# yisol/IDM-VTON

Hardware: AMD Instinct MI355X
Metric: try-on images/sec at 768x1024, 30 DDIM steps, guidance 2.0 (higher is better)
Workload: dtype bf16; 1 GPU; BASELINE.json configs[1]: 768x1024, 30 steps, batch 2/GPU, guidance 2.0, bf16 storage / fp32 accumulate, scheduler ddim, hipGraph on, GarmentNet batched over 6 timesteps, GarmentNet(block b+1)||TryonNet(block b) two-stream overlap on; images_per_call=2, parallelism=dp1 (image shards, one start-up RCCL weight broadcast), rccl_ranks=1

## Files before the change

idm-vton_amd/csrc/gemm_body.cuh:

```cuda
#pragma once
#include <type_traits>
#if !defined(__gfx950__) && !defined(__gfx942__) && defined(__HIP_DEVICE_COMPILE__)
#error "gemm_body.cuh: the counted vmcnt pipeline is written for gfx94x/gfx950 (stores counted in vmcnt)"
#endif
#include "common.cuh"
#include "gemm_common.cuh"

template <typename T, int BN, int BM, int WN, int WM, int ST, bool V1, bool LIN, bool PF, bool TR, bool XA = false>
__device__ __forceinline__ void gemm_body(const GemmParams& p, char* smem, const int m0, const int n0) {
    typedef typename VT<T>::v8 v8;
    typedef typename VT<T>::v4 v4;
    constexpr int NW = WN * WM;
    constexpr int SN = BN / WN, SM = BM / WM;
    constexpr int NI = SN / 32, MI = SM / 32;
    constexpr int WBYTES = BN * 128, XBYTES = BM * 128;
    constexpr int PW_ = BN / 8, PX_ = BM / 8;
    constexpr bool UNEVEN = (PW_ % NW != 0) || (PX_ % NW != 0);
    constexpr int WI = (PW_ + NW - 1) / NW, XI = (PX_ + NW - 1) / NW;
    static_assert(BN % 8 == 0 && BM % 8 == 0 && WN * SN == BN && WM * SM == BM && NI * 32 == SN && MI * 32 == SM, "tile / wave-count mismatch");
    static_assert(!UNEVEN || (V1 && ST == 2), "round-robin piece assignment needs the two-stage ring");
    char* sW = smem;
    char* sX = smem + ST * WBYTES;

    const int lane = threadIdx.x & 63;
    const int wave = uniform(threadIdx.x >> 6);
    const int wn = wave / WM, wm = wave % WM;
    const int u = lane >> 5, l31 = lane & 31;

    const int lrow = lane >> 3, lslot = lane & 7;
    auto wj = [&](int i) { return UNEVEN ? wave + i * NW : wave * WI + i; };
    auto xj = [&](int i) { return UNEVEN ? wave + i * NW : wave * XI + i; };
    uint32_t w_off[WI];
#pragma unroll
    for (int i = 0; i < WI; ++i) {
        const int R = wj(i) * 8 + lrow;
        const int c = lslot ^ ((R >> 1) & 7);
        w_off[i] = ((uint32_t)(n0 + R) * (uint32_t)p.Ktot + c * 8) * 2u;
    }
    int x_pix[XI], x_oy[XI], x_ox[XI], x_c8[XI];
    uint32_t x_off[XI];
    const int HoWo = p.Ho * p.Wo;
    auto kbyte = [&](int t) -> uint32_t { return (uint32_t)t * 128u; };
#pragma unroll
    for (int i = 0; i < XI; ++i) {
        const int R = xj(i) * 8 + lrow;
        const int m = m0 + R;
        x_c8[i] = (lslot ^ ((R >> 1) & 7)) * 8;
        if constexpr (LIN) {
            x_off[i] = m < p.M ? ((uint32_t)m * (uint32_t)p.seg[0].pitch + p.seg[0].coff + x_c8[i]) * 2u : OOB_SENTINEL;
        } else if (m < p.M) {
            const int b = m / HoWo, rem = m - b * HoWo;
            const int oy = rem / p.Wo, ox = rem - oy * p.Wo;
            x_pix[i] = b * p.Hi * p.Wi; x_oy[i] = oy * p.stride; x_ox[i] = ox * p.stride;
        } else {
            x_pix[i] = 0; x_oy[i] = -(1 << 28); x_ox[i] = 0;
        }
    }
    const __amdgpu_buffer_rsrc_t rs_w = make_rsrc(p.w, p.w_bytes);
    const __amdgpu_buffer_rsrc_t rs_x0 = make_rsrc(p.seg[0].ptr, p.seg[0].bytes);
    const int hin = p.ups ? p.Ho : p.Hi, win = p.ups ? p.Wo : p.Wi;

    int si = 0, kseg = 0;
    auto issue = [&](int t, int buf) {
        char* dW = sW + buf * WBYTES;
        char* dX = sX + buf * XBYTES;
#pragma unroll
        for (int i = 0; i < WI; ++i) {
            if (UNEVEN && wj(i) >= PW_) continue;
            dma16(rs_w, dW + wj(i) * 1024, w_off[i] + kbyte(t));
        }
        if constexpr (LIN) {
#pragma unroll
            for (int i = 0; i < XI; ++i) {
                if (UNEVEN && xj(i) >= PX_) continue;
                dma16(rs_x0, dX + xj(i) * 1024, x_off[i] + kbyte(t));
            }
        } else {
            const idmvton_seg sg = p.seg[si];
            const __amdgpu_buffer_rsrc_t rs_x = make_rsrc(sg.ptr, sg.bytes);
#pragma unroll
            for (int i = 0; i < XI; ++i) {
                if (UNEVEN && xj(i) >= PX_) continue;
                int iy = x_oy[i] + sg.dy, ix = x_ox[i] + sg.dx;
                const bool ok = (unsigned)iy < (unsigned)hin && (unsigned)ix < (unsigned)win;
                if (p.ups) { iy >>= 1; ix >>= 1; }
                const uint32_t off = ((uint32_t)(x_pix[i] + iy * p.Wi + ix) * (uint32_t)sg.pitch + sg.coff + kseg + x_c8[i]) * 2u;
                dma16(rs_x, dX + xj(i) * 1024, ok ? off : OOB_SENTINEL);
            }
            kseg += 64;
            if (kseg >= sg.len) { kseg = 0; ++si; }
        }
    };

    idmvton_seg sgc = p.seg[0];
    __amdgpu_buffer_rsrc_t rs_xc = rs_x0;
    auto issue_part = [&](int t, int buf, int s) {
        constexpr int LPT_ = WI + XI;
        char* dW = sW + buf * WBYTES;
        char* dX = sX + buf * XBYTES;
        if constexpr (!LIN) {
            if (s == 0) { sgc = p.seg[si]; rs_xc = make_rsrc(sgc.ptr, sgc.bytes); }
        }
#pragma unroll
        for (int j = 0; j < LPT_; ++j) {
            if ((j & 3) != s) continue;
            if (j < WI) {
                if (UNEVEN && wj(j) >= PW_) continue;
                dma16(rs_w, dW + wj(j) * 1024, w_off[j] + kbyte(t));
            } else {
                const int i = j - WI;
                if (UNEVEN && xj(i) >= PX_) continue;
                if constexpr (LIN) dma16(rs_x0, dX + xj(i) * 1024, x_off[i] + kbyte(t));
                else {
                    int iy = x_oy[i] + sgc.dy, ix = x_ox[i] + sgc.dx;
                    const bool ok = (unsigned)iy < (unsigned)hin && (unsigned)ix < (unsigned)win;
                    if (p.ups) { iy >>= 1; ix >>= 1; }
                    const uint32_t off = ((uint32_t)(x_pix[i] + iy * p.Wi + ix) * (uint32_t)sgc.pitch + sgc.coff + kseg + x_c8[i]) * 2u;
                    dma16(rs_xc, dX + xj(i) * 1024, ok ? off : OOB_SENTINEL);
                }
            }
        }
        if constexpr (!LIN) {
            if (s == 3) { kseg += 64; if (kseg >= sgc.len) { kseg = 0; ++si; } }
        }
    };

    int a_row[NI], a_swz[NI], b_row[MI], b_swz[MI];
#pragma unroll
    for (int ni = 0; ni < NI; ++ni) { const int r = wn * SN + ni * 32 + l31; a_row[ni] = r * 128; a_swz[ni] = (r >> 1) & 7; }
#pragma unroll
    for (int mi = 0; mi < MI; ++mi) { const int r = wm * SM + mi * 32 + l31; b_row[mi] = r * 128; b_swz[mi] = (r >> 1) & 7; }

    f32x16 acc[NI][MI];
#pragma unroll
    for (int ni = 0; ni < NI; ++ni)
#pragma unroll
        for (int mi = 0; mi < MI; ++mi)
#pragma unroll
            for (int r = 0; r < 16; ++r) acc[ni][mi][r] = 0.f;

    auto frag_a = [&](const char* bW, int s, int ni) { return *(const v8*)(bW + a_row[ni] + (((2 * s + u) ^ a_swz[ni]) << 4)); };
    auto frag_b = [&](const char* bX, int s, int mi) { return *(const v8*)(bX + b_row[mi] + (((2 * s + u) ^ b_swz[mi]) << 4)); };
    auto compute = [&](int buf, bool spread = false, int t_next = 0, int buf_next = 0) {
        const char* bW = sW + buf * WBYTES;
        const char* bX = sX + buf * XBYTES;
        if constexpr (!PF) {
#pragma unroll
            for (int s = 0; s < 4; ++s) {
                v8 a[NI], b[MI];
#pragma unroll
                for (int ni = 0; ni < NI; ++ni) a[ni] = frag_a(bW, s, ni);
#pragma unroll
                for (int mi = 0; mi < MI; ++mi) b[mi] = frag_b(bX, s, mi);
                if constexpr (V1) {
                    if (spread) issue_part(t_next, buf_next, s);
                    __builtin_amdgcn_sched_barrier(0);
                }
#pragma unroll
                for (int ni = 0; ni < NI; ++ni)
#pragma unroll
                    for (int mi = 0; mi < MI; ++mi)
                        acc[ni][mi] = TR ? VT<T>::mfma(b[mi], a[ni], acc[ni][mi]) : VT<T>::mfma(a[ni], b[mi], acc[ni][mi]);
            }
        } else {
            v8 a[2][NI], b[2][MI];
#pragma unroll
            for (int ni = 0; ni < NI; ++ni) a[0][ni] = frag_a(bW, 0, ni);
#pragma unroll
            for (int mi = 0; mi < MI; ++mi) b[0][mi] = frag_b(bX, 0, mi);
#pragma unroll
            for (int s = 0; s < 4; ++s) {
                if (s < 3) {
#pragma unroll
                    for (int ni = 0; ni < NI; ++ni) a[(s + 1) & 1][ni] = frag_a(bW, s + 1, ni);
#pragma unroll
                    for (int mi = 0; mi < MI; ++mi) b[(s + 1) & 1][mi] = frag_b(bX, s + 1, mi);
                }
                if (spread) issue_part(t_next, buf_next, s);
                __builtin_amdgcn_sched_barrier(0);
#pragma unroll
                for (int ni = 0; ni < NI; ++ni)
#pragma unroll
                    for (int mi = 0; mi < MI; ++mi)
                        acc[ni][mi] = TR ? VT<T>::mfma(b[s & 1][mi], a[s & 1][ni], acc[ni][mi])
                                         : VT<T>::mfma(a[s & 1][ni], b[s & 1][mi], acc[ni][mi]);
                __builtin_amdgcn_sched_barrier(0);
            }
        }
    };

    v8 xkf[XA ? XA_NK : 1];
    int xa_b = 0, xa_h = 0;
    if constexpr (XA) {
        static_assert(NI == 2 && !TR, "fused cross-attention: one 64-channel head per wave");
        const int mw = m0 + wm * SM;
        xa_b = (mw < p.M ? mw : p.M - 1) / p.xa.tokens;
        xa_h = (n0 + wn * SN) >> 6;
        xattn_load_k<T>(p.xa, xa_b, xa_h, lane, xkf);
    }
    const int nt = p.Ktot >> 6;
    if constexpr (!V1) {
        issue(0, 0);
        for (int t = 0; t < nt; ++t) {
            asm volatile("s_waitcnt vmcnt(0)" ::: "memory");
            __syncthreads();
            if (t + 1 < nt) issue(t + 1, (t + 1) & 1);
            compute(t & 1);
        }
    } else {
        constexpr int LPT = WI + XI;
        static_assert((ST - 2) * LPT < 64, "vmcnt immediate is 6 bits");
#pragma unroll
        for (int s = 0; s < ST - 1; ++s)
            if (s < nt) issue(s, s);
        int cbuf = 0, ibuf = ST - 1;
        for (int t = 0; t < nt; ++t) {
            if (t + ST - 2 < nt) wait_vmcnt<(ST - 2) * LPT>(); else wait_vmcnt<0>();
            __builtin_amdgcn_s_barrier();
            asm volatile("" ::: "memory");
            compute(cbuf, t + ST - 1 < nt, t + ST - 1, ibuf);
            cbuf = cbuf + 1 == ST ? 0 : cbuf + 1;
            ibuf = ibuf + 1 == ST ? 0 : ibuf + 1;
        }
    }

    if constexpr (XA) {
        v8 xvf[XA_NV];
        xattn_load_v<T>(p.xa, xa_b, xa_h, lane, xvf);
        xattn_compute<T, MI>(p.xa, p.M, acc, m0 + wm * SM, lane, xkf, xvf);
    }
    gemm_epilogue<T, NI, MI, SN, SM, TR>(p, acc, m0, n0, wn, wm, lane);
}

template <typename T, int BN, int BM, int WN, int WM, int ST, bool V1, bool LIN, int OCC, bool PFX = false>
__global__ __launch_bounds__(WN * WM * 64, OCC) void gemm_conv_kernel(const GemmParams p) {
    __shared__ __attribute__((aligned(1024))) char smem[ST * (BN + BM) * 128];
    const int wg = xcd_remap(blockIdx.x, p.tiles_m * p.tiles_n);
    int tm, tn;
    if constexpr (!V1) { tm = wg / p.tiles_n; tn = wg - tm * p.tiles_n; }
    else {
        const int GM = p.gm > 0 ? p.gm : 1024 / BM;
        const int width = GM * p.tiles_n;
        const int grp = wg / width, rem = wg - grp * width;
        const int first = grp * GM;
        const int gsz = p.tiles_m - first < GM ? p.tiles_m - first : GM;
        tn = rem / gsz; tm = first + (rem - tn * gsz);
    }
    const int m0 = tm * BM, n0 = tn * BN;
    if constexpr (BN == 320) {
        gemm_body<T, BN, BM, WN, WM, ST, V1, LIN, OCC == 1 || PFX, false>(p, smem, m0, n0);
    } else {
        if (p.vt != nullptr && n0 >= p.vt_n0) gemm_body<T, BN, BM, WN, WM, ST, V1, LIN, OCC == 1 || PFX, true>(p, smem, m0, n0);
        else gemm_body<T, BN, BM, WN, WM, ST, V1, LIN, OCC == 1 || PFX, false>(p, smem, m0, n0);
    }
}

template <typename T, int BN, int BM, int WN, int WM, int ST, int OCC>
__global__ __launch_bounds__(WN * WM * 64, OCC) void gemm_xattn_kernel(const GemmParams p) {
    __shared__ __attribute__((aligned(1024))) char smem[ST * (BN + BM) * 128];
    const int wg = xcd_remap(blockIdx.x, p.tiles_m * p.tiles_n);
    const int GM = p.gm > 0 ? p.gm : 1024 / BM;
    const int width = GM * p.tiles_n;
    const int grp = wg / width, rem = wg - grp * width;
    const int first = grp * GM;
    const int gsz = p.tiles_m - first < GM ? p.tiles_m - first : GM;
    const int tn = rem / gsz, tm = first + (rem - tn * gsz);
    gemm_body<T, BN, BM, WN, WM, ST, true, true, OCC == 1, false, true>(p, smem, tm * BM, tn * BN);
}

template <typename T, int BN, int BM, int WN, int WM, int ST, bool V1, int OCC, bool PFX = false>
static void launch_cfg(const GemmParams& p0, bool lin, hipStream_t st) {
    GemmParams p = p0;
    p.gm = V1 ? idmvton_choose_gm(p.tiles_m, p.tiles_n, BM, BN, p.Ktot) : 0;
    const dim3 grid(p.tiles_n * p.tiles_m), block(WN * WM * 64);
    if constexpr (V1) {
        if (lin) { hipLaunchKernelGGL((gemm_conv_kernel<T, BN, BM, WN, WM, ST, true, true, OCC, PFX>), grid, block, 0, st, p); return; }
    }
    hipLaunchKernelGGL((gemm_conv_kernel<T, BN, BM, WN, WM, ST, V1, false, OCC, PFX>), grid, block, 0, st, p);
}


int gemm_tiles_v0(const GemmParams& p, bool bf16, int bn, int bm, bool lin, hipStream_t st);
int gemm_tiles_v1(const GemmParams& p, bool bf16, int bn, int bm, bool lin, hipStream_t st);
int gemm_tiles_v2(const GemmParams& p, bool bf16, int bn, int bm, bool lin, hipStream_t st);
int gemm_tiles_w8(const GemmParams& p, bool bf16, int bn, int bm, int form, bool lin, hipStream_t st);
int gemm_tiles_xattn(const GemmParams& p, bool bf16, int bn, int bm, int w8, hipStream_t st);
int launch_gemm_lin(const GemmParams& p, bool bf16, int bm, int form, int grid_cap, hipStream_t st);
```

idm-vton_amd/csrc/gemm_common.cuh:

```cuda
#pragma once
#include "common.cuh"
#include "xattn.cuh"

struct GemmParams {
    const void* w; uint32_t w_bytes; int N; int Ktot;
    int nseg; idmvton_seg seg[IDMVTON_MAX_SEG];
    int M, Ho, Wo, Hi, Wi, stride, ups;
    void* out; int ldo;
    const void* bias; const void* rowbias; int rowbias_ld; int rows_per_group;
    const void* res; int ldr;
    int mode;
    void* vt; int vt_n0; int vt_tokens; int vt_perm;
    int colscale_n; float colscale;
    int tiles_m, tiles_n;
    int gm;
    int wide;
    int res32, out32;
    int bias32;
    int out8; float o8_scale, vt8_scale;
    XAttnParams xa;
};

int idmvton_choose_gm(int tiles_m, int tiles_n, int bm, int bn, int K);

template <int N> __device__ __forceinline__ void wait_vmcnt() { asm volatile("s_waitcnt vmcnt(%0)" ::"n"(N) : "memory"); }

__device__ __forceinline__ void swap_cols8(const f32x16& c, const int gp, float (&v)[8]) {
#pragma unroll
    for (int j = 0; j < 4; ++j) {
        const auto r = __builtin_amdgcn_permlane32_swap(__float_as_uint(c[8 * gp + j]), __float_as_uint(c[8 * gp + 4 + j]), false, false);
        v[j] = __uint_as_float(r[0]);
        v[4 + j] = __uint_as_float(r[1]);
    }
}

template <typename T, int NI, int MI, int SN, int SM, bool TR>
__device__ __forceinline__ void gemm_epilogue(const GemmParams& p, f32x16 (&acc)[NI][MI], const int m0, const int n0, const int wn, const int wm,
                                              const int lane) {
    typedef typename VT<T>::v4 v4;
    typedef typename VT<T>::v8 v8;
    const int u = lane >> 5, l31 = lane & 31;
    const T* bias = (const T*)p.bias;
    if constexpr (TR) {
        if (p.out8) {
            uint8_t* vt = (uint8_t*)p.vt;
            const int Cv = p.N - p.vt_n0;
#pragma unroll
            for (int ni = 0; ni < NI; ++ni) {
                const int n = n0 + wn * SN + ni * 32 + l31;
                if (n >= p.N) continue;
                const float bv = bias ? (float)bias[n] : 0.f;
#pragma unroll
                for (int mi = 0; mi < MI; ++mi) {
                    const int m = m0 + wm * SM + mi * 32;
                    if (m >= p.M) continue;
                    const int b = m / p.vt_tokens;
                    const int tok = m - b * p.vt_tokens;
                    int4 o;
                    int w[4];
#pragma unroll
                    for (int g = 0; g < 4; ++g)
                        w[g] = pack4_fp8(clamp448((acc[ni][mi][4 * g] + bv) * p.vt8_scale), clamp448((acc[ni][mi][4 * g + 1] + bv) * p.vt8_scale),
                                         clamp448((acc[ni][mi][4 * g + 2] + bv) * p.vt8_scale), clamp448((acc[ni][mi][4 * g + 3] + bv) * p.vt8_scale));
                    o.x = w[0]; o.y = w[1]; o.z = w[2]; o.w = w[3];
                    *(int4*)(vt + ((size_t)(b * Cv + n - p.vt_n0) * p.vt_tokens + (tok & ~63) + 32 * u + ((tok >> 1) & 16))) = o;
                }
            }
            return;
        }
        if (p.vt_perm) {
            T* vt = (T*)p.vt;
            const int Cv = p.N - p.vt_n0;
#pragma unroll
            for (int ni = 0; ni < NI; ++ni) {
                const int n = n0 + wn * SN + ni * 32 + l31;
                if (n >= p.N) continue;
                const float bv = bias ? (float)bias[n] : 0.f;
#pragma unroll
                for (int mi = 0; mi < MI; ++mi)
#pragma unroll
                    for (int gp = 0; gp < 2; ++gp) {
                        const int m = m0 + wm * SM + mi * 32 + 16 * gp;
                        if (m >= p.M) continue;
                        const int b = m / p.vt_tokens;
                        const int tok = m - b * p.vt_tokens + 8 * u;
                        v8 o;
#pragma unroll
                        for (int j = 0; j < 8; ++j) o[j] = (T)(acc[ni][mi][8 * gp + j] + bv);
                        *(v8*)(vt + ((size_t)(b * Cv + n - p.vt_n0) * p.vt_tokens + tok)) = o;
                    }
            }
            return;
        }
        T* vt = (T*)p.vt;
        const int Cv = p.N - p.vt_n0;
#pragma unroll
        for (int ni = 0; ni < NI; ++ni) {
            const int n = n0 + wn * SN + ni * 32 + l31;
            if (n >= p.N) continue;
            const float bv = bias ? (float)bias[n] : 0.f;
#pragma unroll
            for (int mi = 0; mi < MI; ++mi)
#pragma unroll
                for (int g = 0; g < 4; ++g) {
                    const int m = m0 + wm * SM + mi * 32 + 8 * g + 4 * u;
                    if (m >= p.M) continue;
                    const int b = m / p.vt_tokens;
                    int tok = m - b * p.vt_tokens;
                    if (p.vt_perm) tok = (tok & ~12) | ((tok & 4) << 1) | ((tok & 8) >> 1);
                    v4 o;
#pragma unroll
                    for (int j = 0; j < 4; ++j) o[j] = (T)(acc[ni][mi][4 * g + j] + bv);
                    *(v4*)(vt + ((size_t)(b * Cv + n - p.vt_n0) * p.vt_tokens + tok)) = o;
                }
        }
        return;
    }
    T* out = (T*)p.out;
    const T* res = (const T*)p.res;
    const T* rowbias = (const T*)p.rowbias;
    if (p.wide) {
#pragma unroll
        for (int mi = 0; mi < MI; ++mi) {
            const int m = m0 + wm * SM + mi * 32 + l31;
            if (m >= p.M) continue;
            const T* rb = rowbias ? rowbias + (size_t)(m / p.rows_per_group) * p.rowbias_ld : nullptr;
            if (p.mode == IDMVTON_EPI_GEGLU) {
                if constexpr (NI % 2 == 0) {
#pragma unroll
                    for (int pr = 0; pr < NI / 2; ++pr)
#pragma unroll
                        for (int gp = 0; gp < 2; ++gp) {
                            float h[8], gt[8];
                            swap_cols8(acc[2 * pr][mi], gp, h);
                            swap_cols8(acc[2 * pr + 1][mi], gp, gt);
                            const int nh = n0 + wn * SN + pr * 64 + 16 * gp + 8 * u;
                            if (nh + 32 >= p.N) continue;
                            const int jo = ((n0 + wn * SN + pr * 64) >> 1) + 16 * gp + 8 * u;
                            if (bias) {
                                const v8 bh = *(const v8*)(bias + nh), bg = *(const v8*)(bias + nh + 32);
#pragma unroll
                                for (int j = 0; j < 8; ++j) { h[j] += (float)bh[j]; gt[j] += (float)bg[j]; }
                            }
                            v8 o;
#pragma unroll
                            for (int j = 0; j < 8; ++j) o[j] = (T)(h[j] * gelu_erf(gt[j]));
                            *(v8*)(out + (size_t)m * p.ldo + jo) = o;
                        }
                }
                continue;
            }
#pragma unroll
            for (int ni = 0; ni < NI; ++ni) {
#pragma unroll
                for (int gp = 0; gp < 2; ++gp) {
                    float v[8];
                    swap_cols8(acc[ni][mi], gp, v);
                    const int n = n0 + wn * SN + ni * 32 + 16 * gp + 8 * u;
                    if (n >= p.N) continue;
                    if (bias) {
                        if (p.bias32) {
                            const float4* bp = (const float4*)((const float*)p.bias + n);
                            const float4 b0 = bp[0], b1 = bp[1];
                            v[0] += b0.x; v[1] += b0.y; v[2] += b0.z; v[3] += b0.w;
                            v[4] += b1.x; v[5] += b1.y; v[6] += b1.z; v[7] += b1.w;
                        } else {
                            const v8 bb = *(const v8*)(bias + n);
#pragma unroll
                            for (int j = 0; j < 8; ++j) v[j] += (float)bb[j];
                        }
                    }
                    if (rb) {
                        const v8 bb = *(const v8*)(rb + n);
#pragma unroll
                        for (int j = 0; j < 8; ++j) v[j] += (float)bb[j];
                    }
                    if (n < p.colscale_n) {
#pragma unroll
                        for (int j = 0; j < 8; ++j) v[j] *= p.colscale;
                    }
                    if constexpr (NI * MI <= 8)
                    if (p.out8) {
                        int2 o;
                        o.x = pack4_fp8(clamp448(v[0] * p.o8_scale), clamp448(v[1] * p.o8_scale), clamp448(v[2] * p.o8_scale), clamp448(v[3] * p.o8_scale));
                        o.y = pack4_fp8(clamp448(v[4] * p.o8_scale), clamp448(v[5] * p.o8_scale), clamp448(v[6] * p.o8_scale), clamp448(v[7] * p.o8_scale));
                        *(int2*)((uint8_t*)p.out + (size_t)m * p.ldo + n) = o;
                        continue;
                    }
                    if (p.mode == IDMVTON_EPI_GELU) {
#pragma unroll
                        for (int j = 0; j < 8; ++j) v[j] = gelu_erf(v[j]);
                    } else if (p.mode == IDMVTON_EPI_QUICKGELU) {
#pragma unroll
                        for (int j = 0; j < 8; ++j) v[j] = v[j] / (1.0f + __expf(-1.702f * v[j]));
                    }
                    if (res) {
                        if (p.res32) {
                            const float4* rp = (const float4*)((const float*)p.res + (size_t)m * p.ldr + n);
                            const float4 r0 = rp[0], r1 = rp[1];
                            v[0] += r0.x; v[1] += r0.y; v[2] += r0.z; v[3] += r0.w;
                            v[4] += r1.x; v[5] += r1.y; v[6] += r1.z; v[7] += r1.w;
                        } else {
                            const v8 rr = *(const v8*)(res + (size_t)m * p.ldr + n);
#pragma unroll
                            for (int j = 0; j < 8; ++j) v[j] += (float)rr[j];
                        }
                    }
                    if (p.out32) {
                        float4* op = (float4*)((float*)p.out + (size_t)m * p.ldo + n);
                        op[0] = make_float4(v[0], v[1], v[2], v[3]);
                        op[1] = make_float4(v[4], v[5], v[6], v[7]);
                    } else {
                        v8 o;
#pragma unroll
                        for (int j = 0; j < 8; ++j) o[j] = (T)v[j];
                        *(v8*)(out + (size_t)m * p.ldo + n) = o;
                    }
                }
            }
        }
        return;
    }
    if constexpr (NI * MI <= 8)
#pragma unroll
    for (int mi = 0; mi < MI; ++mi) {
        const int m = m0 + wm * SM + mi * 32 + l31;
        if (m >= p.M) continue;
        const T* rb = rowbias ? rowbias + (size_t)(m / p.rows_per_group) * p.rowbias_ld : nullptr;
        if (p.mode == IDMVTON_EPI_GEGLU) {
            if constexpr (NI % 2 == 0) {
#pragma unroll
                for (int pr = 0; pr < NI / 2; ++pr)
#pragma unroll
                    for (int g = 0; g < 4; ++g) {
                        const int nh = n0 + wn * SN + pr * 64 + 8 * g + 4 * u;
                        if (nh + 32 >= p.N) continue;
                        const int jo = ((n0 + wn * SN + pr * 64) >> 1) + 8 * g + 4 * u;
                        v4 o;
#pragma unroll
                        for (int j = 0; j < 4; ++j) {
                            float h = acc[2 * pr][mi][4 * g + j], gt = acc[2 * pr + 1][mi][4 * g + j];
                            if (bias) { h += (float)bias[nh + j]; gt += (float)bias[nh + 32 + j]; }
                            o[j] = (T)(h * gelu_erf(gt));
                        }
                        *(v4*)(out + (size_t)m * p.ldo + jo) = o;
                    }
            }
            continue;
        }
#pragma unroll
        for (int ni = 0; ni < NI; ++ni)
#pragma unroll
            for (int g = 0; g < 4; ++g) {
                const int n = n0 + wn * SN + ni * 32 + 8 * g + 4 * u;
                if (n >= p.N) continue;
                float v[4];
#pragma unroll
                for (int j = 0; j < 4; ++j) v[j] = acc[ni][mi][4 * g + j];
                if (bias) {
                    const v4 bb = *(const v4*)(bias + n);
#pragma unroll
                    for (int j = 0; j < 4; ++j) v[j] += (float)bb[j];
                }
                if (rb) {
                    const v4 bb = *(const v4*)(rb + n);
#pragma unroll
                    for (int j = 0; j < 4; ++j) v[j] += (float)bb[j];
                }
                if (n < p.colscale_n) {
#pragma unroll
                    for (int j = 0; j < 4; ++j) v[j] *= p.colscale;
                }
                if (p.mode == IDMVTON_EPI_GELU) {
#pragma unroll
                    for (int j = 0; j < 4; ++j) v[j] = gelu_erf(v[j]);
                } else if (p.mode == IDMVTON_EPI_QUICKGELU) {
#pragma unroll
                    for (int j = 0; j < 4; ++j) v[j] = v[j] / (1.0f + __expf(-1.702f * v[j]));
                }
                if (res) {
                    const v4 rr = *(const v4*)(res + (size_t)m * p.ldr + n);
#pragma unroll
                    for (int j = 0; j < 4; ++j) v[j] += (float)rr[j];
                }
                v4 o;
#pragma unroll
                for (int j = 0; j < 4; ++j) o[j] = (T)v[j];
                *(v4*)(out + (size_t)m * p.ldo + n) = o;
            }
    }
}
```

idm-vton_amd/csrc/gemm_conv.hip:

```cpp
#include <cstdlib>
#include <cstring>
#include <vector>
#include "gemm_body.cuh"

int launch_gemm_lin(const GemmParams& p, bool bf16, int bm, int form, int grid_cap, hipStream_t st);

#include <map>
#include <mutex>
#include <tuple>
int idmvton_choose_gm(int tiles_m, int tiles_n, int bm, int bn, int K) {
    static const char* env = getenv("IDMVTON_GM");
    if (env) return atoi(env);
    static const bool model = getenv("IDMVTON_GM_MODEL") && atoi(getenv("IDMVTON_GM_MODEL")) != 0;
    if (!model) return 0;
    static std::mutex mu;
    static std::map<std::tuple<int, int, int, int, int>, int> cache;
    const auto key = std::make_tuple(tiles_m, tiles_n, bm, bn, K);
    std::lock_guard<std::mutex> lk(mu);
    auto it = cache.find(key);
    if (it != cache.end()) return it->second;
    const int T = tiles_m * tiles_n, q = T / 8, r = T % 8;
    static const long cap = getenv("IDMVTON_GM_CAP_KB") ? atol(getenv("IDMVTON_GM_CAP_KB")) << 10 : (2l << 20);
    long best = -1; int best_gm = 0;
    for (int gm = 1; gm <= tiles_m; ++gm) {
        if (gm > 1 && (long)gm * bm * K * 2 > cap) break;
        long cost = 0;
        for (int x = 0; x < 8; ++x) {
            const int lo = x < r ? x * (q + 1) : r * (q + 1) + (x - r) * q, n = x < r ? q + 1 : q;
            int m_lo = tiles_m, m_hi = -1;
            std::vector<char> ms(tiles_m, 0), ns(tiles_n, 0);
            int cm = 0, cn = 0;
            for (int wg = lo; wg < lo + n; ++wg) {
                const int width = gm * tiles_n, grp = wg / width, rem = wg - grp * width, first = grp * gm;
                const int gsz = tiles_m - first < gm ? tiles_m - first : gm;
                const int tn = rem / gsz, tm = first + (rem - tn * gsz);
                if (!ms[tm]) { ms[tm] = 1; ++cm; }
                if (!ns[tn]) { ns[tn] = 1; ++cn; }
            }
            (void)m_lo; (void)m_hi;
            cost += (long)cm * bm + (long)cn * bn;
        }
        if (best < 0 || cost < best) { best = cost; best_gm = gm; }
    }
    cache[key] = best_gm;
    return best_gm;
}

static int launch_gemm(const GemmParams& p0, bool bf16, int variant, int bn, int bm, bool lin, hipStream_t st) {
    GemmParams p = p0;
    int form = 0;
    int grid_cap = 0;
    if (variant == 5) { form = bm & 15; grid_cap = (bm & 0x4000) ? 5 : 0; bm &= ~(15 | 0x4000); }
    p.tiles_n = (p.N + bn - 1) / bn;
    p.tiles_m = (p.M + bm - 1) / bm;
    int rc = 1;
    if (p.mode == IDMVTON_EPI_XATTN) {
        if (bm != 64 && p.xa.tokens % 64 != 0) {
            bm = 64;
            p.tiles_m = (p.M + bm - 1) / bm;
        }
        if (gemm_tiles_xattn(p, bf16, bn, bm, variant == 6 && bn == 128 && bm == 128, st))
            return idmvton_set_error(IDMVTON_E_ARG, "gemm_conv: IDMVTON_EPI_XATTN runs on the 128x64, 128x128 and 128x256 tiles (got %dx%d)", bn, bm);
        CHECK_LAUNCH("gemm_conv");
        return IDMVTON_OK;
    }
    if (variant == 0) rc = gemm_tiles_v0(p, bf16, bn, bm, lin, st);
    else if (variant == 1) rc = gemm_tiles_v1(p, bf16, bn, bm, lin, st);
    else if (variant == 2) rc = gemm_tiles_v2(p, bf16, bn, bm, lin, st);
    else if (variant == 5) {
        if (!(bn == 256 && (bm == 256 || bm == 192))) return idmvton_set_error(IDMVTON_E_ARG, "gemm_conv: variant 5 is the 256x256 / 256x192 tile");
        if (lin) rc = launch_gemm_lin(p, bf16, bm, form, grid_cap, st);
        else if (bm == 256) rc = gemm_tiles_v1(p, bf16, 256, 256, lin, st);
        else {
            p.tiles_n = (p.N + 127) / 128; p.tiles_m = (p.M + 255) / 256;
            rc = gemm_tiles_v1(p, bf16, 128, 256, lin, st);
        }
    } else if (variant == 6) {
        const int form6 = bm & 15;
        bm &= ~15;
        p.tiles_m = (p.M + bm - 1) / bm;
        if (bn == 320 && (p.vt || !p.wide || p.out8 || p.mode == IDMVTON_EPI_GEGLU)) {
            const int fbn = bn == 320 ? 128 : bn, fbm = bn == 320 ? 256 : bm;
            p.tiles_n = (p.N + fbn - 1) / fbn;
            p.tiles_m = (p.M + fbm - 1) / fbm;
            rc = gemm_tiles_v1(p, bf16, fbn, fbm, lin, st);
        } else rc = gemm_tiles_w8(p, bf16, bn, bm, form6, lin, st);
    } else return idmvton_set_error(IDMVTON_E_ARG, "gemm_conv: unknown variant %d", variant);
    if (rc) return idmvton_set_error(IDMVTON_E_ARG, "gemm_conv: variant %d has no %dx%d tile", variant, bn, bm);
    CHECK_LAUNCH("gemm_conv");
    return IDMVTON_OK;
}

extern "C" int idmvton_gemm_conv(const idmvton_gemm_conv_args* a, void* stream) {
    CHECK_ARG(a != nullptr, IDMVTON_E_ARG, "gemm_conv: null args");
    CHECK_ARG(a->dtype == IDMVTON_F16 || a->dtype == IDMVTON_BF16, IDMVTON_E_DTYPE, "gemm_conv: dtype %d", a->dtype);
    CHECK_ARG(a->M > 0 && a->N > 0 && a->Ktot > 0, IDMVTON_E_SHAPE, "gemm_conv: M=%d N=%d K=%d", a->M, a->N, a->Ktot);
    CHECK_ARG(a->Ktot % 64 == 0, IDMVTON_E_SHAPE, "gemm_conv: Ktot=%d must be a multiple of 64", a->Ktot);
    CHECK_ARG(a->N % 4 == 0, IDMVTON_E_SHAPE, "gemm_conv: N=%d must be a multiple of 4", a->N);
    CHECK_ARG(a->nseg >= 1 && a->nseg <= IDMVTON_MAX_SEG, IDMVTON_E_SHAPE, "gemm_conv: nseg=%d", a->nseg);
    int ksum = 0;
    for (int s = 0; s < a->nseg; ++s) {
        const idmvton_seg& g = a->seg[s];
        CHECK_ARG(g.ptr && g.len > 0 && g.len % 64 == 0, IDMVTON_E_SHAPE, "gemm_conv: seg %d len=%d", s, g.len);
        CHECK_ARG(g.pitch % 8 == 0 && g.coff % 8 == 0, IDMVTON_E_ALIGN, "gemm_conv: seg %d pitch=%d coff=%d", s, g.pitch, g.coff);
        CHECK_ARG(g.bytes < 0x80000000u, IDMVTON_E_SHAPE, "gemm_conv: seg %d tensor >= 2 GiB", s);
        CHECK_ARG(((uintptr_t)g.ptr & 15) == 0, IDMVTON_E_ALIGN, "gemm_conv: seg %d pointer not 16-byte aligned", s);
        ksum += g.len;
    }
    CHECK_ARG(ksum == a->Ktot, IDMVTON_E_SHAPE, "gemm_conv: segment lengths sum to %d, Ktot=%d", ksum, a->Ktot);
    CHECK_ARG(a->Ho > 0 && a->Wo > 0 && a->Hi > 0 && a->Wi > 0 && a->stride > 0 && a->M % (a->Ho * a->Wo) == 0,
              IDMVTON_E_SHAPE, "gemm_conv: geometry M=%d Ho=%d Wo=%d", a->M, a->Ho, a->Wo);
    if (a->ups) CHECK_ARG(a->stride == 1 && a->Ho <= 2 * a->Hi && a->Ho >= 2 * a->Hi - 1 && a->Wo <= 2 * a->Wi && a->Wo >= 2 * a->Wi - 1, IDMVTON_E_SHAPE,
                          "gemm_conv: ups=1 needs stride 1 and an output grid of 2Hi x 2Wi or one short of it (Ho=%d Hi=%d Wo=%d Wi=%d)", a->Ho, a->Hi, a->Wo, a->Wi);
    CHECK_ARG(a->w && ((uintptr_t)a->w & 15) == 0, IDMVTON_E_ALIGN, "gemm_conv: weight pointer");
    const uint64_t wbytes = (uint64_t)a->N * a->Ktot * 2;
    CHECK_ARG(wbytes + (uint64_t)128 * a->Ktot * 2 < 0xFFFFFFFFull, IDMVTON_E_SHAPE, "gemm_conv: weight too large");
    const bool geglu = a->mode == IDMVTON_EPI_GEGLU, xattn = a->mode == IDMVTON_EPI_XATTN;
    CHECK_ARG(a->mode == IDMVTON_EPI_NONE || a->mode == IDMVTON_EPI_GELU || a->mode == IDMVTON_EPI_QUICKGELU || geglu || xattn, IDMVTON_E_ARG, "gemm_conv: mode %d", a->mode);
    CHECK_ARG(a->colscale_n >= 0 && a->colscale_n % 4 == 0 && !(geglu && a->colscale_n), IDMVTON_E_ARG, "gemm_conv: colscale_n=%d", a->colscale_n);
    if (geglu) CHECK_ARG(a->N % 64 == 0 && !a->res && !a->rowbias && !a->vt, IDMVTON_E_ARG, "gemm_conv: GEGLU needs N%%64==0, no res/rowbias/vt");
    CHECK_ARG(a->out || (a->vt && a->vt_n0 == 0), IDMVTON_E_ARG, "gemm_conv: null out");
    if (a->out) CHECK_ARG(a->ldo % 4 == 0 && ((uintptr_t)a->out & 7) == 0, IDMVTON_E_ALIGN, "gemm_conv: out alignment");
    if (a->res) CHECK_ARG(a->ldr % 4 == 0 && ((uintptr_t)a->res & 7) == 0, IDMVTON_E_ALIGN, "gemm_conv: res alignment");
    if (a->bias) CHECK_ARG(((uintptr_t)a->bias & 7) == 0, IDMVTON_E_ALIGN, "gemm_conv: bias alignment");
    if (a->rowbias) CHECK_ARG(a->rowbias_ld % 4 == 0 && a->rows_per_group > 0 && ((uintptr_t)a->rowbias & 7) == 0,
                              IDMVTON_E_ALIGN, "gemm_conv: rowbias");
    if (a->vt && a->vt_perm) CHECK_ARG(((uintptr_t)a->vt & 15) == 0, IDMVTON_E_ALIGN, "gemm_conv: vt pointer not 16-byte aligned");
    if (a->vt && a->vt_perm) CHECK_ARG(a->vt_tokens % 16 == 0, IDMVTON_E_ARG, "gemm_conv: vt_perm needs vt_tokens %% 16 == 0 (got %d)", a->vt_tokens);
    if (a->vt) CHECK_ARG(a->vt_tokens > 0 && a->vt_tokens % 4 == 0 && a->M % a->vt_tokens == 0 && a->vt_n0 % 64 == 0 &&
                         a->vt_n0 >= 0 && a->vt_n0 < a->N && ((uintptr_t)a->vt & 7) == 0,
                         IDMVTON_E_ARG, "gemm_conv: vt_tokens=%d vt_n0=%d", a->vt_tokens, a->vt_n0);

    GemmParams p;
    memset(&p.xa, 0, sizeof(p.xa));
    if (xattn) {
        const idmvton_xattn* x = a->xattn;
        CHECK_ARG(x != nullptr && (x->nseg == 1 || x->nseg == 2), IDMVTON_E_ARG, "gemm_conv: IDMVTON_EPI_XATTN needs `xattn` with 1 or 2 key segments");
        CHECK_ARG(a->N % 64 == 0 && !a->bias && !a->res && !a->rowbias && !a->vt && !a->colscale_n && !a->io_flags &&
                  a->nseg == 1 && a->Ho == 1 && a->Hi == 1 && a->Wo == a->M && a->Wi == a->M && a->out && a->ldo % 8 == 0 && ((uintptr_t)a->out & 15) == 0,
                  IDMVTON_E_ARG, "gemm_conv: IDMVTON_EPI_XATTN is a plain Linear with N %% 64 == 0 and nothing else in its epilogue");
        CHECK_ARG(x->tokens > 0 && x->tokens % 32 == 0 && a->M % x->tokens == 0, IDMVTON_E_SHAPE, "gemm_conv: xattn.tokens=%d (rows per batch element, a multiple of 32 dividing M=%d)", x->tokens, a->M);
        for (int s = 0; s < x->nseg; ++s) {
            const int nk_max = s == 0 ? 96 : 32;
            CHECK_ARG(x->k[s] && x->vt[s] && x->nk[s] > 0 && x->nk[s] <= nk_max && x->k_rows[s] >= ((x->nk[s] + 31) & ~31) && x->ldk[s] >= a->N && x->ldk[s] % 8 == 0 &&
                      x->ldvt[s] >= ((x->nk[s] + 15) & ~15) && x->ldvt[s] % 8 == 0 && (((uintptr_t)x->k[s] | (uintptr_t)x->vt[s]) & 15) == 0, IDMVTON_E_SHAPE,
                      "gemm_conv: xattn segment %d: nk=%d (<= %d) k_rows=%d (>= round32(nk)) ldk=%d ldvt=%d (>= round16(nk))", s, x->nk[s], nk_max, x->k_rows[s], x->ldk[s], x->ldvt[s]);
            p.xa.k[s] = x->k[s]; p.xa.vt[s] = x->vt[s]; p.xa.ldk[s] = x->ldk[s]; p.xa.ldvt[s] = x->ldvt[s]; p.xa.nk[s] = x->nk[s]; p.xa.krows[s] = x->k_rows[s];
        }
        p.xa.nseg = x->nseg; p.xa.tokens = x->tokens; p.xa.vchan = a->N; p.xa.ip_scale = x->ip_scale;
    } else CHECK_ARG(a->xattn == nullptr, IDMVTON_E_ARG, "gemm_conv: `xattn` without mode IDMVTON_EPI_XATTN");
    p.w = a->w; p.w_bytes = (uint32_t)wbytes; p.N = a->N; p.Ktot = a->Ktot;
    p.nseg = a->nseg;
    for (int s = 0; s < IDMVTON_MAX_SEG; ++s) p.seg[s] = a->seg[s < a->nseg ? s : a->nseg - 1];
    p.M = a->M; p.Ho = a->Ho; p.Wo = a->Wo; p.Hi = a->Hi; p.Wi = a->Wi; p.stride = a->stride; p.ups = a->ups ? 1 : 0;
    p.out = a->out; p.ldo = a->ldo; p.bias = a->bias; p.rowbias = a->rowbias; p.rowbias_ld = a->rowbias_ld;
    p.rows_per_group = a->rows_per_group > 0 ? a->rows_per_group : 1; p.res = a->res; p.ldr = a->ldr; p.mode = a->mode;
    p.vt = a->vt; p.vt_n0 = a->vt_n0; p.vt_tokens = a->vt_tokens > 0 ? a->vt_tokens : 4; p.vt_perm = a->vt_perm ? 1 : 0;
    p.colscale_n = a->colscale_n; p.colscale = a->colscale;
    p.tiles_m = p.tiles_n = 0; p.gm = 0;
    {
        auto a16 = [](const void* q) { return ((uintptr_t)q & 15) == 0; };
        const int n_out = geglu ? a->N / 2 : a->N;
        p.wide = n_out % 8 == 0 && a->N % 8 == 0 && a->colscale_n % 8 == 0 && (!a->out || (a->ldo % 8 == 0 && a16(a->out))) &&
                 (!a->res || (a->ldr % 8 == 0 && a16(a->res))) && (!a->bias || a16(a->bias)) &&
                 (!a->rowbias || (a->rowbias_ld % 8 == 0 && a16(a->rowbias))) && (!a->vt || a->vt_n0 % 8 == 0);
    }

    int variant = 1, bn = 64, bm = 64;
    static const bool env_narrow = getenv("IDMVTON_EPILOGUE_8B") != nullptr;
    if ((a->tile_hint & 0x8000) || env_narrow) p.wide = 0;
    p.res32 = (a->io_flags & IDMVTON_IO_RES_F32) ? 1 : 0;
    p.out32 = (a->io_flags & IDMVTON_IO_OUT_F32) ? 1 : 0;
    p.bias32 = (a->io_flags & IDMVTON_IO_BIAS_F32) ? 1 : 0;
    if (p.bias32) CHECK_ARG(a->bias && p.wide && !geglu && !a->vt && ((uintptr_t)a->bias & 15) == 0, IDMVTON_E_ARG,
                            "gemm_conv: IDMVTON_IO_BIAS_F32 needs a 16-byte aligned bias and the plain 16-byte epilogue (no GEGLU, no vt)");
    CHECK_ARG((a->io_flags & ~15) == 0, IDMVTON_E_ARG, "gemm_conv: io_flags=%d", a->io_flags);
    p.out8 = (a->io_flags & IDMVTON_IO_OUT_F8) ? 1 : 0;
    p.o8_scale = a->f8_out_scale; p.vt8_scale = a->f8_vt_scale;
    if (p.out8) {
        CHECK_ARG(a->io_flags == IDMVTON_IO_OUT_F8 && a->mode == IDMVTON_EPI_NONE && !a->res && !a->rowbias && p.wide,
                  IDMVTON_E_ARG, "gemm_conv: IDMVTON_IO_OUT_F8 needs the plain 16-byte epilogue (no activation / residual / rowbias / fp32 IO)");
        CHECK_ARG((!a->out || a->f8_out_scale > 0.f) && (!a->vt || (a->f8_vt_scale > 0.f && a->vt_tokens % 64 == 0 && ((uintptr_t)a->vt & 15) == 0)),
                  IDMVTON_E_ARG, "gemm_conv: IDMVTON_IO_OUT_F8: scales > 0, vt_tokens %% 64 == 0 (got %d), 16-byte aligned vt", a->vt_tokens);
    }
    if (p.res32 || p.out32) {
        CHECK_ARG((a->io_flags & ~7) == 0 && !geglu && !a->vt, IDMVTON_E_ARG, "gemm_conv: io_flags=%d (fp32 res / out: no GEGLU, no vt)", a->io_flags);
        CHECK_ARG(!p.res32 || a->res, IDMVTON_E_ARG, "gemm_conv: IDMVTON_IO_RES_F32 without res");
        CHECK_ARG(p.wide, IDMVTON_E_ALIGN, "gemm_conv: the fp32 residual stream needs the 16-byte epilogue (N, ldo, ldr multiples of 8, 16-byte aligned pointers)");
    }
    if (a->tile_hint) { variant = (a->tile_hint >> 28) & 0xf; bn = (a->tile_hint >> 16) & 0xfff; bm = a->tile_hint & 0x7fff; }
    else {
        static const int cand[5][2] = {{256, 256}, {128, 256}, {128, 128}, {128, 64}, {64, 64}};
        for (int i = 0; i < 5; ++i) {
            const int n_ = cand[i][0], m_ = cand[i][1];
            if (geglu && n_ < 128) continue;
            if (xattn && (n_ != 128)) continue;
            if (a->vt && a->vt_n0 % n_ != 0) continue;
            if (i < 4 && (n_ > ((a->N + 63) & ~63) || m_ > ((a->M + 63) & ~63))) continue;
            bn = n_; bm = m_;
            if ((long)((a->N + n_ - 1) / n_) * ((a->M + m_ - 1) / m_) >= 200) break;
        }
    }
    if (geglu) CHECK_ARG(bn >= 128, IDMVTON_E_ARG, "gemm_conv: GEGLU needs BN >= 128 (64-row wave tiles)");
    if (a->vt) CHECK_ARG(a->vt_n0 % bn == 0, IDMVTON_E_ARG, "gemm_conv: vt_n0 %% BN != 0");
    const idmvton_seg& s0 = a->seg[0];
    const bool lin = a->nseg == 1 && a->Ho == 1 && a->Hi == 1 && a->Wo == a->M && a->Wi == a->M && a->stride == 1 &&
                     !a->ups && s0.dy == 0 && s0.dx == 0 && (uint64_t)a->M * s0.pitch * 2 < 0x80000000ull;
    if (!a->tile_hint && bn == 256 && bm == 256 && lin) { variant = 5; bm = 257; }
    else if (!a->tile_hint && !xattn) {
        if (bn == 256 && bm == 256) variant = 6;
        else if (bn == 128 && bm == 128) variant = 6;
        if (a->N > 256 && a->N <= 320 && p.wide && !a->vt && !geglu && !p.out8 && (a->M + 191) / 192 >= 200) { variant = 6; bn = 320; bm = 192; }
    }
    hipStream_t st = (hipStream_t)stream;
    return launch_gemm(p, a->dtype == IDMVTON_BF16, variant, bn, bm, lin, st);
}
```

Before: 1.592 images/s.

## Add slab loader for 3x3 stride-1 convs reusing one row slab across dx taps

New measurement: 1.595 images/s (median of 6 runs). No clear change (+0.2%).

```diff
diff --git a/idm-vton_amd/csrc/conv_slab_index.h b/idm-vton_amd/csrc/conv_slab_index.h
--- /dev/null
+++ b/idm-vton_amd/csrc/conv_slab_index.h
@@ -0,0 +1,45 @@
+#pragma once
+
+namespace conv_slab {
+
+constexpr int SLICE = 64;
+
+constexpr int pieces(int bm) { return bm / 8 + 1; }
+constexpr int rows(int bm) { return pieces(bm) * 8; }
+
+constexpr int row(int r, int dx) { return r + 1 + dx; }
+
+constexpr int row_pixel(int m0, int R) { return m0 + R - 1; }
+
+constexpr int pixel_oy(int m, int H, int W) { return (m % (H * W)) / W; }
+constexpr int pixel_ox(int m, int W) { return m % W; }
+
+constexpr bool row_valid(int m0, int R, int dy, int H, int W, int M) {
+    const int m = row_pixel(m0, R);
+    return m >= 0 && m < M && pixel_oy(m, H, W) + dy >= 0 && pixel_oy(m, H, W) + dy < H;
+}
+constexpr int row_source(int m0, int R, int dy, int W) { return row_pixel(m0, R) + dy * W; }
+
+constexpr bool edge_lo(int ox) { return ox == 0; }
+constexpr bool edge_hi(int ox, int W) { return ox == W - 1; }
+constexpr bool tap_is_zero(int ox, int dx, int W) { return (dx < 0 && edge_lo(ox)) || (dx > 0 && edge_hi(ox, W)); }
+
+constexpr int ktiles(int C) { return 9 * (C / SLICE); }
+constexpr int koff(int s, int t, int C) { return t * C + SLICE * s; }
+constexpr int ktile_slice(int kt) { return kt / 9; }
+constexpr int ktile_tap(int kt) { return kt % 9; }
+
+template <typename Seg>
+constexpr bool eligible(const Seg* seg, int nseg, int stride, int ups, int Ho, int Wo, int Hi, int Wi) {
+    if (nseg < 9 || stride != 1 || ups || Ho != Hi || Wo != Wi) return false;
+    for (int t = 0; t < 9; ++t) {
+        const Seg& g = seg[t];
+        if (g.ptr != seg[0].ptr || g.bytes != seg[0].bytes || g.pitch != seg[0].pitch || g.coff != seg[0].coff || g.len != seg[0].len) return false;
+        if (g.dy != t / 3 - 1 || g.dx != t % 3 - 1) return false;
+    }
+    for (int t = 9; t < nseg; ++t)
+        if (seg[t].dy != 0 || seg[t].dx != 0) return false;
+    return seg[0].len % SLICE == 0;
+}
+
+}
diff --git a/idm-vton_amd/csrc/gemm_body.cuh b/idm-vton_amd/csrc/gemm_body.cuh
--- a/idm-vton_amd/csrc/gemm_body.cuh
+++ b/idm-vton_amd/csrc/gemm_body.cuh
@@ -5,11 +5,27 @@
 #endif
 #include "common.cuh"
 #include "gemm_common.cuh"
-
-template <typename T, int BN, int BM, int WN, int WM, int ST, bool V1, bool LIN, bool PF, bool TR, bool XA = false>
+#include "conv_slab_index.h"
+
+enum { LD_GATHER = 0, LD_LIN = 1, LD_SLAB = 2 };
+
+constexpr int slab_part_min(int ph, int SI, int SPREAD, int NW, int PS) {
+    int n = 0;
+    for (int i = 0; i < SI; ++i) n += (ph < SPREAD && i % SPREAD == ph && NW - 1 + i * NW < PS) ? 1 : 0;
+    return n;
+}
+constexpr int slab_steady_vmcnt(int ph, int ST, int WI, int SI, int SPREAD, int NW, int PS) {
+    int n = 0;
+    for (int j = 1; j <= ST - 2; ++j) n += WI + slab_part_min((ph - j + 6) % 3, SI, SPREAD, NW, PS);
+    return n;
+}
+template <int V> struct ic { static constexpr int value = V; };
+
+template <typename T, int BN, int BM, int WN, int WM, int ST, bool V1, int LD, bool PF, bool TR, bool XA = false>
 __device__ __forceinline__ void gemm_body(const GemmParams& p, char* smem, const int m0, const int n0) {
     typedef typename VT<T>::v8 v8;
     typedef typename VT<T>::v4 v4;
+    constexpr bool LIN = LD == LD_LIN, SLAB = LD == LD_SLAB;
     constexpr int NW = WN * WM;
     constexpr int SN = BN / WN, SM = BM / WM;
     constexpr int NI = SN / 32, MI = SM / 32;
@@ -19,6 +35,7 @@
     constexpr int WI = (PW_ + NW - 1) / NW, XI = (PX_ + NW - 1) / NW;
     static_assert(BN % 8 == 0 && BM % 8 == 0 && WN * SN == BN && WM * SM == BM && NI * 32 == SN && MI * 32 == SM, "tile / wave-count mismatch");
     static_assert(!UNEVEN || (V1 && ST == 2), "round-robin piece assignment needs the two-stage ring");
+    constexpr int PS = conv_slab::pieces(BM), SI = (PS + NW - 1) / NW, SBYTES = PS * 1024;
     char* sW = smem;
     char* sX = smem + ST * WBYTES;
 
@@ -46,7 +63,8 @@
         const int R = xj(i) * 8 + lrow;
         const int m = m0 + R;
         x_c8[i] = (lslot ^ ((R >> 1) & 7)) * 8;
-        if constexpr (LIN) {
+        if constexpr (SLAB) {
+        } else if constexpr (LIN) {
             x_off[i] = m < p.M ? ((uint32_t)m * (uint32_t)p.seg[0].pitch + p.seg[0].coff + x_c8[i]) * 2u : OOB_SENTINEL;
         } else if (m < p.M) {
             const int b = m / HoWo, rem = m - b * HoWo;
@@ -199,7 +217,194 @@
         xattn_load_k<T>(p.xa, xa_b, xa_h, lane, xkf);
     }
     const int nt = p.Ktot >> 6;
-    if constexpr (!V1) {
+    if constexpr (SLAB) {
+        namespace cs = conv_slab;
+        static_assert(ST >= 2 && ST <= 4 && !XA, "slab loader: ring of 2 to 4 weight stages");
+        constexpr int SPREAD = 5 - ST;
+        const idmvton_seg sg0 = p.seg[0];
+        const int H = p.Ho, W = p.Wo, C = sg0.len;
+        const int nslab = cs::ktiles(C), G = nslab / 3;
+        auto sj = [&](int i) { return wave + i * NW; };
+        uint32_t s_off[SI];
+        int s_oy[SI];
+#pragma unroll
+        for (int i = 0; i < SI; ++i) {
+            const int R = sj(i) * 8 + lrow;
+            const int m = cs::row_pixel(m0, R);
+            if ((unsigned)m < (unsigned)p.M) {
+                s_oy[i] = cs::pixel_oy(m, H, W);
+                s_off[i] = ((uint32_t)m * (uint32_t)sg0.pitch + sg0.coff + (lslot ^ ((R >> 1) & 7)) * 8) * 2u;
+            } else { s_oy[i] = -(1 << 28); s_off[i] = 0; }
+        }
+        int b_r[MI];
+        uint32_t e_lo = 0, e_hi = 0;
+#pragma unroll
+        for (int mi = 0; mi < MI; ++mi) {
+            b_r[mi] = wm * SM + mi * 32 + l31;
+            const int ox = cs::pixel_ox(m0 + b_r[mi], W);
+            e_lo |= (cs::edge_lo(ox) ? 1u : 0u) << mi;
+            e_hi |= (cs::edge_hi(ox, W) ? 1u : 0u) << mi;
+        }
+        const bool any_lo = __builtin_amdgcn_ballot_w64(e_lo != 0) != 0, any_hi = __builtin_amdgcn_ballot_w64(e_hi != 0) != 0;
+
+        int g_dy = -1, g_sl = 0, gi = 0;
+        auto issue_slab = [&](int buf, int ph, int s, bool all) {
+            char* dS = sX + buf * SBYTES;
+            const uint32_t gofs = (uint32_t)((g_dy * W * sg0.pitch + cs::SLICE * g_sl) * 2);
+#pragma unroll
+            for (int i = 0; i < SI; ++i) {
+                if (!all && (i % SPREAD != ph || ((i / SPREAD) & 3) != s)) continue;
+                if (sj(i) >= PS) continue;
+                const bool ok = (unsigned)(s_oy[i] + g_dy) < (unsigned)H;
+                dma16(rs_x0, dS + sj(i) * 1024, ok ? s_off[i] + gofs : OOB_SENTINEL);
+            }
+        };
+        auto slab_advance = [&] { ++gi; if (++g_dy > 1) { g_dy = -1; ++g_sl; } };
+        int w_t = 0, w_sl = 0, w_tap = 0;
+        auto issue_w = [&](int buf, int s, int mask) {
+            const uint32_t kb = w_t < nslab ? (uint32_t)cs::koff(w_sl, w_tap, C) * 2u : kbyte(w_t);
+            char* dW = sW + buf * WBYTES;
+#pragma unroll
+            for (int j = 0; j < WI; ++j) {
+                if ((j & mask) != s) continue;
+                if (UNEVEN && wj(j) >= PW_) continue;
+                dma16(rs_w, dW + wj(j) * 1024, w_off[j] + kb);
+            }
+        };
+        auto w_advance = [&] { ++w_t; if (++w_tap == 9) { w_tap = 0; ++w_sl; } };
+        si = 9;
+        auto issue_tail = [&](int buf, int s) {
+            if (s == 0) { sgc = p.seg[si]; rs_xc = make_rsrc(sgc.ptr, sgc.bytes); }
+            char* dS = sX + buf * SBYTES;
+#pragma unroll
+            for (int i = 0; i < XI; ++i) {
+                if ((i & 1) != s) continue;
+                if (UNEVEN && xj(i) >= PX_) continue;
+                const int R = xj(i) * 8 + lrow, m = m0 + R;
+                const uint32_t off = ((uint32_t)m * (uint32_t)sgc.pitch + sgc.coff + kseg + (lslot ^ ((R >> 1) & 7)) * 8) * 2u;
+                dma16(rs_xc, dS + xj(i) * 1024, m < p.M ? off : OOB_SENTINEL);
+            }
+            if (s == 1) { kseg += 64; if (kseg >= sgc.len) { kseg = 0; ++si; } }
+        };
+
+        auto frag_base = [&](int mi, int sh) { const int R = b_r[mi] + sh; return R * 128 + ((u ^ ((R >> 1) & 7)) << 4); };
+        auto frag_s = [&](const char* bS, int s, int base) { return *(const v8*)(bS + (base ^ (s << 5))); };
+        auto edge_fix = [&](auto PHC, v8 (&b)[MI]) {
+            constexpr int PH = decltype(PHC)::value;
+            if constexpr (PH == 0 || PH == 2) {
+                const uint32_t e = PH == 0 ? e_lo : e_hi;
+                if (PH == 0 ? any_lo : any_hi) {
+#pragma unroll
+                    for (int mi = 0; mi < MI; ++mi) {
+                        const u32x4 v = __builtin_bit_cast(u32x4, b[mi]);
+                        const u32x4 z = {0u, 0u, 0u, 0u};
+                        b[mi] = __builtin_bit_cast(v8, ((e >> mi) & 1u) ? z : v);
+                    }
+                }
+            }
+        };
+        auto compute_s = [&](auto PHC, int wbuf, int sbuf, auto&& hook) {
+            constexpr int PH = decltype(PHC)::value;
+            constexpr int SH = PH == 3 ? 0 : cs::row(0, PH - 1);
+            const char* bW = sW + wbuf * WBYTES;
+            const char* bS = sX + sbuf * SBYTES;
+            int fb[MI];
+#pragma unroll
+            for (int mi = 0; mi < MI; ++mi) fb[mi] = frag_base(mi, SH);
+            if constexpr (!PF) {
+#pragma unroll
+                for (int s = 0; s < 4; ++s) {
+                    v8 a[NI], b[MI];
+#pragma unroll
+                    for (int ni = 0; ni < NI; ++ni) a[ni] = frag_a(bW, s, ni);
+#pragma unroll
+                    for (int mi = 0; mi < MI; ++mi) b[mi] = frag_s(bS, s, fb[mi]);
+                    if constexpr (V1) {
+                        hook(s);
+                        __builtin_amdgcn_sched_barrier(0);
+                    }
+                    edge_fix(PHC, b);
+#pragma unroll
+                    for (int ni = 0; ni < NI; ++ni)
+#pragma unroll
+                        for (int mi = 0; mi < MI; ++mi)
+                            acc[ni][mi] = TR ? VT<T>::mfma(b[mi], a[ni], acc[ni][mi]) : VT<T>::mfma(a[ni], b[mi], acc[ni][mi]);
+                }
+            } else {
+                v8 a[2][NI], b[2][MI];
+#pragma unroll
+                for (int ni = 0; ni < NI; ++ni) a[0][ni] = frag_a(bW, 0, ni);
+#pragma unroll
+                for (int mi = 0; mi < MI; ++mi) b[0][mi] = frag_s(bS, 0, fb[mi]);
+#pragma unroll
+                for (int s = 0; s < 4; ++s) {
+                    if (s < 3) {
+#pragma unroll
+                        for (int ni = 0; ni < NI; ++ni) a[(s + 1) & 1][ni] = frag_a(bW, s + 1, ni);
+#pragma unroll
+                        for (int mi = 0; mi < MI; ++mi) b[(s + 1) & 1][mi] = frag_s(bS, s + 1, fb[mi]);
+                    }
+                    if constexpr (V1) hook(s);
+                    __builtin_amdgcn_sched_barrier(0);
+                    edge_fix(PHC, b[s & 1]);
+#pragma unroll
+                    for (int ni = 0; ni < NI; ++ni)
+#pragma unroll
+                        for (int mi = 0; mi < MI; ++mi)
+                            acc[ni][mi] = TR ? VT<T>::mfma(b[s & 1][mi], a[s & 1][ni], acc[ni][mi])
+                                             : VT<T>::mfma(a[s & 1][ni], b[s & 1][mi], acc[ni][mi]);
+                    __builtin_amdgcn_sched_barrier(0);
+                }
+            }
+        };
+
+        issue_slab(0, 0, 0, true);
+        slab_advance();
+#pragma unroll
+        for (int s = 0; s < ST - 1; ++s) { issue_w(s, 0, 0); w_advance(); }
+        int t = 0, cbuf = 0, ibuf = ST - 1, sbuf = 0;
+        auto ktile = [&](auto PHC) {
+            constexpr int PH = decltype(PHC)::value;
+            if constexpr (!V1) {
+                wait_vmcnt<0>();
+                __syncthreads();
+            } else {
+                if (PH < 3 && t <= nslab - 3) wait_vmcnt<slab_steady_vmcnt(PH % 3, ST, WI, SI, SPREAD, NW, PS)>();
+                else if (t + ST - 2 < nt) wait_vmcnt<(ST >= 3 ? WI : 0)>();
+                else wait_vmcnt<0>();
+                __builtin_amdgcn_s_barrier();
+                asm volatile("" ::: "memory");
+            }
+            const bool has_w = t + ST - 1 < nt;
+            const bool tail_next = PH >= 2 && t + 1 >= nslab && t + 1 < nt;
+            const bool slab_next = PH < SPREAD && gi < G;
+            auto hook = [&](int s) {
+                if (PH >= 2 && tail_next) {
+                    if (s < 2) issue_tail(sbuf ^ 1, s);
+                    else if (has_w) issue_w(ibuf, s - 2, 1);
+                } else {
+                    if (has_w) issue_w(ibuf, s, 3);
+                    if constexpr (PH < SPREAD) { if (slab_next) issue_slab(sbuf ^ 1, PH, s, false); }
+                }
+                if (s == 3) {
+                    if (has_w) w_advance();
+                    if constexpr (PH == SPREAD - 1) { if (slab_next) slab_advance(); }
+                }
+            };
+            if constexpr (V1) compute_s(PHC, cbuf, sbuf, hook);
+            else {
+#pragma unroll
+                for (int s = 0; s < 4; ++s) hook(s);
+                compute_s(PHC, cbuf, sbuf, hook);
+            }
+            cbuf = cbuf + 1 == ST ? 0 : cbuf + 1;
+            ibuf = ibuf + 1 == ST ? 0 : ibuf + 1;
+            if constexpr (PH >= 2) sbuf ^= 1;
+            ++t;
+        };
+        for (int g = 0; g < G; ++g) { ktile(ic<0>{}); ktile(ic<1>{}); ktile(ic<2>{}); }
+        while (t < nt) ktile(ic<3>{});
+    } else if constexpr (!V1) {
         issue(0, 0);
         for (int t = 0; t < nt; ++t) {
             asm volatile("s_waitcnt vmcnt(0)" ::: "memory");
@@ -232,9 +437,9 @@
     gemm_epilogue<T, NI, MI, SN, SM, TR>(p, acc, m0, n0, wn, wm, lane);
 }
 
-template <typename T, int BN, int BM, int WN, int WM, int ST, bool V1, bool LIN, int OCC, bool PFX = false>
+template <typename T, int BN, int BM, int WN, int WM, int ST, bool V1, int LD, int OCC, bool PFX = false>
 __global__ __launch_bounds__(WN * WM * 64, OCC) void gemm_conv_kernel(const GemmParams p) {
-    __shared__ __attribute__((aligned(1024))) char smem[ST * (BN + BM) * 128];
+    __shared__ __attribute__((aligned(1024))) char smem[LD == LD_SLAB ? ST * BN * 128 + 2 * conv_slab::pieces(BM) * 1024 : ST * (BN + BM) * 128];
     const int wg = xcd_remap(blockIdx.x, p.tiles_m * p.tiles_n);
     int tm, tn;
     if constexpr (!V1) { tm = wg / p.tiles_n; tn = wg - tm * p.tiles_n; }
@@ -248,10 +453,10 @@
     }
     const int m0 = tm * BM, n0 = tn * BN;
     if constexpr (BN == 320) {
-        gemm_body<T, BN, BM, WN, WM, ST, V1, LIN, OCC == 1 || PFX, false>(p, smem, m0, n0);
+        gemm_body<T, BN, BM, WN, WM, ST, V1, LD, OCC == 1 || PFX, false>(p, smem, m0, n0);
     } else {
-        if (p.vt != nullptr && n0 >= p.vt_n0) gemm_body<T, BN, BM, WN, WM, ST, V1, LIN, OCC == 1 || PFX, true>(p, smem, m0, n0);
-        else gemm_body<T, BN, BM, WN, WM, ST, V1, LIN, OCC == 1 || PFX, false>(p, smem, m0, n0);
+        if (p.vt != nullptr && n0 >= p.vt_n0) gemm_body<T, BN, BM, WN, WM, ST, V1, LD, OCC == 1 || PFX, true>(p, smem, m0, n0);
+        else gemm_body<T, BN, BM, WN, WM, ST, V1, LD, OCC == 1 || PFX, false>(p, smem, m0, n0);
     }
 }
 
@@ -265,7 +470,7 @@
     const int first = grp * GM;
     const int gsz = p.tiles_m - first < GM ? p.tiles_m - first : GM;
     const int tn = rem / gsz, tm = first + (rem - tn * gsz);
-    gemm_body<T, BN, BM, WN, WM, ST, true, true, OCC == 1, false, true>(p, smem, tm * BM, tn * BN);
+    gemm_body<T, BN, BM, WN, WM, ST, true, LD_LIN, OCC == 1, false, true>(p, smem, tm * BM, tn * BN);
 }
 
 template <typename T, int BN, int BM, int WN, int WM, int ST, bool V1, int OCC, bool PFX = false>
@@ -273,10 +478,11 @@
     GemmParams p = p0;
     p.gm = V1 ? idmvton_choose_gm(p.tiles_m, p.tiles_n, BM, BN, p.Ktot) : 0;
     const dim3 grid(p.tiles_n * p.tiles_m), block(WN * WM * 64);
+    if (p.slab) { hipLaunchKernelGGL((gemm_conv_kernel<T, BN, BM, WN, WM, ST, V1, LD_SLAB, OCC, PFX>), grid, block, 0, st, p); return; }
     if constexpr (V1) {
-        if (lin) { hipLaunchKernelGGL((gemm_conv_kernel<T, BN, BM, WN, WM, ST, true, true, OCC, PFX>), grid, block, 0, st, p); return; }
-    }
-    hipLaunchKernelGGL((gemm_conv_kernel<T, BN, BM, WN, WM, ST, V1, false, OCC, PFX>), grid, block, 0, st, p);
+        if (lin) { hipLaunchKernelGGL((gemm_conv_kernel<T, BN, BM, WN, WM, ST, true, LD_LIN, OCC, PFX>), grid, block, 0, st, p); return; }
+    }
+    hipLaunchKernelGGL((gemm_conv_kernel<T, BN, BM, WN, WM, ST, V1, LD_GATHER, OCC, PFX>), grid, block, 0, st, p);
 }
 
 
diff --git a/idm-vton_amd/csrc/gemm_common.cuh b/idm-vton_amd/csrc/gemm_common.cuh
--- a/idm-vton_amd/csrc/gemm_common.cuh
+++ b/idm-vton_amd/csrc/gemm_common.cuh
@@ -6,6 +6,7 @@
     const void* w; uint32_t w_bytes; int N; int Ktot;
     int nseg; idmvton_seg seg[IDMVTON_MAX_SEG];
     int M, Ho, Wo, Hi, Wi, stride, ups;
+    int slab;
     void* out; int ldo;
     const void* bias; const void* rowbias; int rowbias_ld; int rows_per_group;
     const void* res; int ldr;
diff --git a/idm-vton_amd/csrc/gemm_conv.hip b/idm-vton_amd/csrc/gemm_conv.hip
--- a/idm-vton_amd/csrc/gemm_conv.hip
+++ b/idm-vton_amd/csrc/gemm_conv.hip
@@ -153,6 +153,7 @@
     p.nseg = a->nseg;
     for (int s = 0; s < IDMVTON_MAX_SEG; ++s) p.seg[s] = a->seg[s < a->nseg ? s : a->nseg - 1];
     p.M = a->M; p.Ho = a->Ho; p.Wo = a->Wo; p.Hi = a->Hi; p.Wi = a->Wi; p.stride = a->stride; p.ups = a->ups ? 1 : 0;
+    p.slab = conv_slab::eligible(a->seg, a->nseg, a->stride, a->ups ? 1 : 0, a->Ho, a->Wo, a->Hi, a->Wi) ? 1 : 0;
     p.out = a->out; p.ldo = a->ldo; p.bias = a->bias; p.rowbias = a->rowbias; p.rowbias_ld = a->rowbias_ld;
     p.rows_per_group = a->rows_per_group > 0 ? a->rows_per_group : 1; p.res = a->res; p.ldr = a->ldr; p.mode = a->mode;
     p.vt = a->vt; p.vt_n0 = a->vt_n0; p.vt_tokens = a->vt_tokens > 0 ? a->vt_tokens : 4; p.vt_perm = a->vt_perm ? 1 : 0;
```
